# marksgraham/ddpm-ood

Measured on AMD Instinct MI355X. Metric: reconstructions/sec (whole node), FashionMNIST 32x32, higher is better.
Workload: dtype f32 (split-f16 MFMA products, fp32 accumulate)

## Files before the change

ddpm_ood_amd/csrc/conv_direct.hip:

```cpp
#include <stdlib.h>

#include "common.h"

namespace ddpm {

template <int COB>
__global__ __launch_bounds__(256) void conv_direct_kernel(const ddpm_conv_desc a) {
  const int HWo = a.Ho * a.Wo, HWi = a.Hi * a.Wi;
  const int Cin = a.C1 + a.C2;
  const int T = a.ksize * a.ksize;
  const int pad = a.ksize == 3 ? 1 : 0;
  const int s = a.mode == DDPM_CONV_STRIDE2 ? 2 : 1;
  const bool up = a.mode == DDPM_CONV_UPSAMPLE2;
  const int Hv = up ? a.Ho : a.Hi, Wv = up ? a.Wo : a.Wi;

  const int p = blockIdx.x * 256 + threadIdx.x;
  const int n = blockIdx.z;
  const int co0 = blockIdx.y * COB;
  if (p >= HWo) return;
  const int ho = p / a.Wo, wo = p - ho * a.Wo;

  float acc[COB];
#pragma unroll
  for (int j = 0; j < COB; ++j) acc[j] = 0.f;

  for (int ci = 0; ci < Cin; ++ci) {
    const float *plane = (ci < a.C1) ? a.in1 + ((size_t)n * a.C1 + ci) * HWi
                                     : a.in2 + ((size_t)n * a.C2 + (ci - a.C1)) * HWi;
    float sc = 1.f, sh = 0.f;
    if (a.gscale) {
      sc = a.gscale[(size_t)n * Cin + ci];
      sh = a.gshift[(size_t)n * Cin + ci];
    }
    for (int kh = 0; kh < a.ksize; ++kh) {
      for (int kw = 0; kw < a.ksize; ++kw) {
        const int hv = ho * s + kh - pad, wv = wo * s + kw - pad;
        float v = 0.f;
        if (hv >= 0 && hv < Hv && wv >= 0 && wv < Wv) {
          v = up ? plane[(hv >> 1) * a.Wi + (wv >> 1)] : plane[hv * a.Wi + wv];
          if (a.gscale) v = v * sc + sh;
          if (a.act == DDPM_ACT_SILU) v = silu_fast(v);
          if (a.act == DDPM_ACT_RELU) v = fmaxf(v, 0.f);
        }
        const int t = kh * a.ksize + kw;
#pragma unroll
        for (int j = 0; j < COB; ++j) {
          const int co = (co0 + j < a.Cout) ? co0 + j : a.Cout - 1;
          acc[j] = fmaf(v, a.w_raw[((size_t)co * Cin + ci) * T + t], acc[j]);
        }
      }
    }
  }
#pragma unroll
  for (int j = 0; j < COB; ++j) {
    const int co = co0 + j;
    if (co < a.Cout) {
      const size_t idx = ((size_t)n * a.Cout + co) * HWo + p;
      float v = acc[j];
      if (a.bias) v += a.bias[co];
      if (a.chan_add) v += a.chan_add[(size_t)n * a.chan_add_stride + co];
      if (a.residual) v += a.residual[idx];
      if (a.out_act == DDPM_ACT_RELU) v = fmaxf(v, 0.f);
      a.out[idx] = v;
    }
  }
}

constexpr int kSC_CH = 8;

template <int NPOS>
__global__ __launch_bounds__(256) void conv_smallco_kernel(const ddpm_conv_desc a, int TH, int RS, int PS) {
  extern __shared__ __attribute__((aligned(16))) float tile[];
  const int HW = a.Ho * a.Wo;
  const int Cin = a.C1 + a.C2;
  const int tid = threadIdx.x;
  const int n = blockIdx.y;
  const int h0 = blockIdx.x * TH;
  const bool live = tid < TH * a.Wo;
  const int th = live ? tid / a.Wo : 0, tw = live ? tid - th * a.Wo : 0;

  int soff[NPOS];
#pragma unroll
  for (int j = 0; j < NPOS; ++j) {
    const int r = tid + 256 * j;
    soff[j] = -1;
    if (r < PS) {
      const int ir = r / RS, ic = r - ir * RS;
      const int hv = h0 + ir - 1, wv = ic - 1;
      if (hv >= 0 && hv < a.Hi && wv >= 0 && wv < a.Wi) soff[j] = hv * a.Wi + wv;
    }
  }
  float acc[4] = {0.f, 0.f, 0.f, 0.f};
  const int pix = th * RS + tw;

  float pre[NPOS][kSC_CH], psc[kSC_CH], psh[kSC_CH];
  auto fetch = [&](int c0) {
#pragma unroll
    for (int c = 0; c < kSC_CH; ++c) {
      const int ci = c0 + c;
      const bool okc = ci < Cin;
      const float *plane = !okc ? a.in1
                           : (ci < a.C1) ? a.in1 + ((size_t)n * a.C1 + ci) * HW
                                         : a.in2 + ((size_t)n * a.C2 + (ci - a.C1)) * HW;
#pragma unroll
      for (int j = 0; j < NPOS; ++j) pre[j][c] = (okc && soff[j] >= 0) ? plane[soff[j]] : 0.f;
      psc[c] = (okc && a.gscale) ? a.gscale[(size_t)n * Cin + ci] : 1.f;
      psh[c] = (okc && a.gscale) ? a.gshift[(size_t)n * Cin + ci] : 0.f;
    }
  };
  fetch(0);
  for (int c0 = 0; c0 < Cin; c0 += kSC_CH) {
    __syncthreads();
#pragma unroll
    for (int j = 0; j < NPOS; ++j) {
      const int r = tid + 256 * j;
      if (r < PS) {
#pragma unroll
        for (int c = 0; c < kSC_CH; ++c) {
          float v = 0.f;
          if (soff[j] >= 0 && c0 + c < Cin) {
            v = pre[j][c];
            if (a.gscale) v = v * psc[c] + psh[c];
            if (a.act == DDPM_ACT_SILU) v = silu_fast(v);
            if (a.act == DDPM_ACT_RELU) v = fmaxf(v, 0.f);
          }
          tile[c * PS + r] = v;
        }
      }
    }
    __syncthreads();
    if (c0 + kSC_CH < Cin) fetch(c0 + kSC_CH);
#pragma unroll
    for (int c = 0; c < kSC_CH; ++c) {
      const int ci = c0 + c;
      if (ci < Cin) {
        float x[9];
#pragma unroll
        for (int kh = 0; kh < 3; ++kh)
#pragma unroll
          for (int kw = 0; kw < 3; ++kw) x[kh * 3 + kw] = tile[c * PS + pix + kh * RS + kw];
        for (int co = 0; co < a.Cout; ++co) {
          const float *w = a.w_raw + ((size_t)co * Cin + ci) * 9;
#pragma unroll
          for (int t = 0; t < 9; ++t) acc[co] = fmaf(x[t], w[t], acc[co]);
        }
      }
    }
  }
  const int p = (h0 + th) * a.Wo + tw;
  for (int co = 0; co < a.Cout && live; ++co) {
    const size_t idx = ((size_t)n * a.Cout + co) * HW + p;
    float v = acc[co];
    if (a.bias) v += a.bias[co];
    if (a.chan_add) v += a.chan_add[(size_t)n * a.chan_add_stride + co];
    if (a.residual) v += a.residual[idx];
    if (a.out_act == DDPM_ACT_RELU) v = fmaxf(v, 0.f);
    a.out[idx] = v;
  }
}

constexpr int kSW_NJ = 7;
constexpr int kSW_PPL = 4;

template <int NWV>
__global__ __launch_bounds__(64 * NWV) void conv_smallco_wave_kernel(const ddpm_conv_desc a, int TH, int RS, int PS) {
  extern __shared__ __attribute__((aligned(16))) float lds[];
  const int HW = a.Ho * a.Wo;
  const int Cin = a.C1 + a.C2;
  const int tid = threadIdx.x, lane = tid & 63, wave = __builtin_amdgcn_readfirstlane(tid >> 6);
  const int n = blockIdx.y;
  const int h0 = blockIdx.x * TH;
  float *plane_lds = lds + wave * 2 * PS;

  int soff[kSW_NJ];
#pragma unroll
  for (int j = 0; j < kSW_NJ; ++j) {
    const int r = lane + 64 * j;
    soff[j] = -1;
    if (r < PS) {
      const int ir = r / RS, ic = r - ir * RS;
      const int hv = h0 + ir - 1, wv = ic - 1;
      if (hv >= 0 && hv < a.Hi && wv >= 0 && wv < a.Wi) soff[j] = hv * a.Wi + wv;
    }
  }
  int pix[kSW_PPL];
#pragma unroll
  for (int k = 0; k < kSW_PPL; ++k) {
    const int q = lane + 64 * k;
    const int th = q / a.Wo, tw = q - th * a.Wo;
    pix[k] = (q < TH * a.Wo) ? th * RS + tw : 0;
  }
  float acc[kSW_PPL][4];
#pragma unroll
  for (int k = 0; k < kSW_PPL; ++k)
#pragma unroll
    for (int c = 0; c < 4; ++c) acc[k][c] = 0.f;

  float pre[2][kSW_NJ], psc[2] = {1.f, 1.f}, psh[2] = {0.f, 0.f};
  auto fetch = [&](int slot, int ci) {
    const float *plane = (ci < a.C1) ? a.in1 + ((size_t)n * a.C1 + ci) * HW
                                     : a.in2 + ((size_t)n * a.C2 + (ci - a.C1)) * HW;
#pragma unroll
    for (int j = 0; j < kSW_NJ; ++j) pre[slot][j] = soff[j] >= 0 ? plane[soff[j]] : 0.f;
    if (a.gscale) {
      psc[slot] = a.gscale[(size_t)n * Cin + ci];
      psh[slot] = a.gshift[(size_t)n * Cin + ci];
    }
  };
  auto consume = [&](int slot, int ci, int buf) {
    float *pl = plane_lds + buf * PS;
#pragma unroll
    for (int j = 0; j < kSW_NJ; ++j) {
      const int r = lane + 64 * j;
      if (r < PS) {
        float v = 0.f;
        if (soff[j] >= 0) {
          v = pre[slot][j];
          if (a.gscale) v = v * psc[slot] + psh[slot];
          if (a.act == DDPM_ACT_SILU) v = silu_fast(v);
          if (a.act == DDPM_ACT_RELU) v = fmaxf(v, 0.f);
        }
        pl[r] = v;
      }
    }
    if (ci + 2 * NWV < Cin) fetch(slot, ci + 2 * NWV);
    float wreg[4][9];
#pragma unroll
    for (int co = 0; co < 4; ++co) {
      const float *w = a.w_raw + ((size_t)min(co, a.Cout - 1) * Cin + ci) * 9;
#pragma unroll
      for (int t = 0; t < 9; ++t) wreg[co][t] = w[t];
    }
#pragma unroll
    for (int k = 0; k < kSW_PPL; ++k) {
      float x[9];
#pragma unroll
      for (int kh = 0; kh < 3; ++kh)
#pragma unroll
        for (int kw = 0; kw < 3; ++kw) x[kh * 3 + kw] = pl[pix[k] + kh * RS + kw];
#pragma unroll
      for (int co = 0; co < 4; ++co)
        if (co < a.Cout) {
#pragma unroll
          for (int t = 0; t < 9; ++t) acc[k][co] = fmaf(x[t], wreg[co][t], acc[k][co]);
        }
    }
  };
  if (wave < Cin) fetch(0, wave);
  if (wave + NWV < Cin) fetch(1, wave + NWV);
  for (int ci = wave; ci < Cin; ci += 2 * NWV) {
    consume(0, ci, 0);
    if (ci + NWV < Cin) consume(1, ci + NWV, 1);
  }
  float *red = lds + NWV * 2 * PS;
#pragma unroll
  for (int k = 0; k < kSW_PPL; ++k)
#pragma unroll
    for (int c = 0; c < 4; ++c) red[(wave * 256 + lane + 64 * k) * 4 + c] = acc[k][c];
  __syncthreads();
  if (tid < TH * a.Wo) {
    const int th = tid / a.Wo, tw = tid - th * a.Wo;
    const int p = (h0 + th) * a.Wo + tw;
    for (int co = 0; co < a.Cout; ++co) {
      float v = red[(0 * 256 + tid) * 4 + co];
#pragma unroll
      for (int wv = 1; wv < NWV; ++wv) v += red[(wv * 256 + tid) * 4 + co];
      const size_t idx = ((size_t)n * a.Cout + co) * HW + p;
      if (a.bias) v += a.bias[co];
      if (a.chan_add) v += a.chan_add[(size_t)n * a.chan_add_stride + co];
      if (a.residual) v += a.residual[idx];
      if (a.out_act == DDPM_ACT_RELU) v = fmaxf(v, 0.f);
      a.out[idx] = v;
    }
  }
}

template <int CIN>
__global__ __launch_bounds__(256) void conv_smallci_kernel(const ddpm_conv_desc a) {
  const int HW = a.Ho * a.Wo;
  const int p = blockIdx.x * 256 + threadIdx.x;
  const int n = blockIdx.y;
  if (p >= HW) return;
  const int ho = p / a.Wo, wo = p - ho * a.Wo;
  float x[CIN * 9];
#pragma unroll
  for (int ci = 0; ci < CIN; ++ci) {
    const float *plane = a.in1 + ((size_t)n * CIN + ci) * HW;
#pragma unroll
    for (int kh = 0; kh < 3; ++kh)
#pragma unroll
      for (int kw = 0; kw < 3; ++kw) {
        const int hv = ho + kh - 1, wv = wo + kw - 1;
        x[ci * 9 + kh * 3 + kw] = (hv >= 0 && hv < a.Hi && wv >= 0 && wv < a.Wi) ? plane[hv * a.Wi + wv] : 0.f;
      }
  }
  float *dst = a.out + (size_t)n * a.Cout * HW + p;
  const int cpz = (a.Cout + gridDim.z - 1) / gridDim.z, co_end = min(a.Cout, ((int)blockIdx.z + 1) * cpz);
  extern __shared__ float2 wred[];
  const bool emit = a.stats_out != nullptr;
  const int lane = threadIdx.x & 63, wave = threadIdx.x >> 6;
#pragma unroll 4
  for (int co = blockIdx.z * cpz; co < co_end; ++co) {
    const float *w = a.w_raw + (size_t)co * CIN * 9;
    float acc = 0.f;
#pragma unroll
    for (int k = 0; k < CIN * 9; ++k) acc = fmaf(x[k], w[k], acc);
    if (a.bias) acc += a.bias[co];
    dst[(size_t)co * HW] = acc;
    if (emit) {
      const float mean = wave_sum_dpp_last_lane(acc);
      const float mu = __builtin_bit_cast(float, __builtin_amdgcn_readlane(__builtin_bit_cast(int, mean), 63)) * (1.f / 64.f);
      const float dv = acc - mu;
      const float q = wave_sum_dpp_last_lane(dv * dv);
      if (lane == 63) wred[(co - blockIdx.z * cpz) * 4 + wave] = make_float2(mu, q);
    }
  }
  if (emit) {
    __syncthreads();
    const int parts = HW / 256;
    for (int c = threadIdx.x; c < co_end - (int)blockIdx.z * cpz; c += 256) {
      const float2 w0 = wred[c * 4], w1 = wred[c * 4 + 1], w2 = wred[c * 4 + 2], w3 = wred[c * 4 + 3];
      const float m01 = 0.5f * (w0.x + w1.x), d01 = w1.x - w0.x, q01 = (w0.y + w1.y) + d01 * d01 * 32.f;
      const float m23 = 0.5f * (w2.x + w3.x), d23 = w3.x - w2.x, q23 = (w2.y + w3.y) + d23 * d23 * 32.f;
      const float mm = 0.5f * (m01 + m23), dd = m23 - m01, qq = (q01 + q23) + dd * dd * 64.f;
      const int co = blockIdx.z * cpz + c;
      *reinterpret_cast<float2 *>(a.stats_out + (((size_t)n * a.Cout + co) * parts + blockIdx.x) * 2) = make_float2(mm, qq);
    }
  }
}

static bool smallci_supported(const ddpm_conv_desc &d) {
  const bool on = sw().convin_fast;
  return on && d.C2 == 0 && d.C1 >= 1 && d.C1 <= 4 && d.ksize == 3 && d.mode == DDPM_CONV_NORMAL && !d.gscale &&
         d.act == DDPM_ACT_NONE && !d.chan_add && !d.residual && d.out_act == DDPM_ACT_NONE && d.Cout >= 16 &&
         d.Di <= 1 && d.Do <= 1 && d.dims != 3;
}

static int smallci_stats_parts(const ddpm_conv_desc &d) {
  const int HW = d.Ho * d.Wo;
  if (!smallci_supported(d) || HW % 256 || HW / 256 > 8) return 0;
  return HW / 256;
}

static bool smallco_supported(const ddpm_conv_desc &d, int &TH, int &RS, int &PS) {
  if (d.Cout > 4 || d.ksize != 3 || d.mode != DDPM_CONV_NORMAL || d.Wo > 256 || d.Di > 1 || d.Do > 1) return false;
  TH = 0;
  for (int th = 256 / d.Wo; th >= 1; --th)
    if (d.Ho % th == 0) { TH = th; break; }
  if (TH == 0 || 2 * TH * d.Wo < 256) return false;
  RS = d.Wo + 2;
  PS = (TH + 2) * RS;
  return PS <= 512;
}

int launch_conv_direct(const ddpm_conv_desc &d, hipStream_t s) {
  DDPM_CHECK_ARG(d.w_raw != nullptr, "conv_direct: w_raw is NULL");
  DDPM_CHECK_ARG(d.ksize == 1 || d.ksize == 3, "conv_direct: ksize must be 1 or 3");
  DDPM_CHECK_ARG(d.B <= 65535, "conv_direct: batch > 65535");
  const int HWo = d.Ho * d.Wo;
  const double cin = d.C1 + d.C2, taps = d.ksize * d.ksize;
  const int Cin_i = d.C1 + d.C2;
  int TH, RS, PS;
  if (smallco_supported(d, TH, RS, PS)) {
    ProfScope prof(s, "conv3x3_small_cout", 2.0 * d.B * HWo * d.Cout * cin * 9,
                   4.0 * ((double)d.B * cin * HWo + (double)d.B * HWo * d.Cout + d.Cout * cin * 9));
    dim3 grid(d.Ho / TH, d.B);
    const bool wave_ok = sw().convout_wave;
    if (wave_ok && PS <= 64 * kSW_NJ && Cin_i >= 16) {
      const long w16_max = sw().convout_w16_maxwg;
      const long w16_wgs = w16_max >= 0 ? w16_max : 2L * device_cus();
      if ((long)grid.x * grid.y <= w16_wgs && Cin_i >= 64) {
        const size_t lds_w = ((size_t)16 * 2 * PS + 16 * 256 * 4) * sizeof(float);
        static bool attr_done = false;
        if (!attr_done) {
          (void)hipFuncSetAttribute(reinterpret_cast<const void *>(&conv_smallco_wave_kernel<16>), hipFuncAttributeMaxDynamicSharedMemorySize, 160 * 1024);
          attr_done = true;
        }
        hipLaunchKernelGGL(conv_smallco_wave_kernel<16>, grid, dim3(1024), lds_w, s, d, TH, RS, PS);
        DDPM_CHECK_LAUNCH();
        return 0;
      }
      const size_t lds_w = ((size_t)4 * 2 * PS + 4 * 256 * 4) * sizeof(float);
      hipLaunchKernelGGL(conv_smallco_wave_kernel<4>, grid, dim3(256), lds_w, s, d, TH, RS, PS);
      DDPM_CHECK_LAUNCH();
      return 0;
    }
    const size_t lds = (size_t)kSC_CH * PS * sizeof(float);
    if (PS <= 256)
      hipLaunchKernelGGL(conv_smallco_kernel<1>, grid, dim3(256), lds, s, d, TH, RS, PS);
    else
      hipLaunchKernelGGL(conv_smallco_kernel<2>, grid, dim3(256), lds, s, d, TH, RS, PS);
    DDPM_CHECK_LAUNCH();
    return 0;
  }
  if (smallci_supported(d)) {
    ProfScope prof(s, "conv3x3_small_cin", 2.0 * d.B * HWo * d.Cout * cin * 9,
                   4.0 * ((double)d.B * cin * HWo + (double)d.B * HWo * d.Cout + d.Cout * cin * 9));
    const long blocks = (long)((HWo + 255) / 256) * d.B;
    int zs = 1;
    const long zblk = sw().convin_blocks_per_cu;
    while (zs < 8 && blocks * zs * 2 <= device_cus() * zblk && d.Cout / (zs * 2) >= 16) zs *= 2;
    dim3 grid((HWo + 255) / 256, d.B, zs);
    ddpm_conv_desc dk = d;
    if (smallci_stats_parts(d) == 0) dk.stats_out = nullptr;
    const size_t lds = dk.stats_out ? (size_t)((d.Cout + zs - 1) / zs) * 4 * sizeof(float2) : 0;
    switch (d.C1) {
      case 1: hipLaunchKernelGGL(conv_smallci_kernel<1>, grid, dim3(256), lds, s, dk); break;
      case 2: hipLaunchKernelGGL(conv_smallci_kernel<2>, grid, dim3(256), lds, s, dk); break;
      case 3: hipLaunchKernelGGL(conv_smallci_kernel<3>, grid, dim3(256), lds, s, dk); break;
      default: hipLaunchKernelGGL(conv_smallci_kernel<4>, grid, dim3(256), lds, s, dk); break;
    }
    DDPM_CHECK_LAUNCH();
    return 0;
  }
  ProfScope prof(s, "conv_direct", 2.0 * d.B * HWo * d.Cout * cin * taps,
                 4.0 * ((double)d.B * cin * d.Hi * d.Wi + (double)d.B * HWo * d.Cout * (d.residual ? 2 : 1) +
                        d.Cout * cin * taps));
  if (d.Cout <= 4) {
    dim3 grid((HWo + 255) / 256, d.Cout, d.B);
    hipLaunchKernelGGL(conv_direct_kernel<1>, grid, dim3(256), 0, s, d);
  } else {
    dim3 grid((HWo + 255) / 256, (d.Cout + 7) / 8, d.B);
    hipLaunchKernelGGL(conv_direct_kernel<8>, grid, dim3(256), 0, s, d);
  }
  DDPM_CHECK_LAUNCH();
  return 0;
}

bool conv_direct_supported(const ddpm_conv_desc &) { return true; }

int conv_direct_stats_parts(const ddpm_conv_desc &d) {
  int TH, RS, PS;
  return d.mode == DDPM_CONV_NORMAL && !smallco_supported(d, TH, RS, PS) ? smallci_stats_parts(d) : 0;
}

}
```

Baseline: 1058.

## Add quad-pixel small-Cin conv kernel with LDS weights and per-wave channel split

Adds a new kernel for the 3x3 small-input-channel conv (the network's input layer). Each lane computes four adjacent output pixels from a register-held 3x6 input window. The block's output channels are split across its four waves, and weights plus bias are staged in LDS. The aim is to reuse input loads across pixels and channels and to store with float4. Per-channel mean/variance stats are reduced inside one wave over 256 pixels, which removes the cross-wave LDS merge. The cost is more registers per thread and reliance on Wo being a multiple of 4.

```diff
diff --git a/ddpm_ood_amd/csrc/conv_direct.hip b/ddpm_ood_amd/csrc/conv_direct.hip
--- a/ddpm_ood_amd/csrc/conv_direct.hip
+++ b/ddpm_ood_amd/csrc/conv_direct.hip
@@ -325,6 +325,92 @@
       const float mm = 0.5f * (m01 + m23), dd = m23 - m01, qq = (q01 + q23) + dd * dd * 64.f;
       const int co = blockIdx.z * cpz + c;
       *reinterpret_cast<float2 *>(a.stats_out + (((size_t)n * a.Cout + co) * parts + blockIdx.x) * 2) = make_float2(mm, qq);
+    }
+  }
+}
+
+template <int CIN>
+__global__ __launch_bounds__(256) void conv_smallci_quad_kernel(const ddpm_conv_desc a) {
+  constexpr int K = CIN * 9;
+  constexpr int U = CIN == 1 ? 4 : CIN == 2 ? 2 : 1;
+  const int HW = a.Ho * a.Wo;
+  const int lane = threadIdx.x & 63, wave = __builtin_amdgcn_readfirstlane(threadIdx.x >> 6);
+  const int p = blockIdx.x * 256 + 4 * lane;
+  const int n = blockIdx.y;
+  const int cpz = (a.Cout + gridDim.z - 1) / gridDim.z, z0 = blockIdx.z * cpz, z_end = min(a.Cout, z0 + cpz);
+  extern __shared__ __attribute__((aligned(16))) float wlds[];
+  for (int i = threadIdx.x; i < (z_end - z0) * (K + 1); i += 256) {
+    const int c = i / (K + 1), k = i - c * (K + 1);
+    wlds[i] = k < K ? a.w_raw[(size_t)(z0 + c) * K + k] : (a.bias ? a.bias[z0 + c] : 0.f);
+  }
+  __syncthreads();
+  if (p >= HW) return;
+  const int ho = p / a.Wo, wo = p - ho * a.Wo;
+  float x[CIN][3][6];
+#pragma unroll
+  for (int ci = 0; ci < CIN; ++ci) {
+    const float *plane = a.in1 + ((size_t)n * CIN + ci) * HW;
+#pragma unroll
+    for (int kh = 0; kh < 3; ++kh)
+#pragma unroll
+      for (int c = 0; c < 6; ++c) {
+        const int hv = ho + kh - 1, wv = wo + c - 1;
+        const bool ok = hv >= 0 && hv < a.Hi && wv >= 0 && wv < a.Wi;
+        const float v = plane[ok ? hv * a.Wi + wv : p];
+        x[ci][kh][c] = ok ? v : 0.f;
+      }
+  }
+  const int cpw = (z_end - z0 + 3) / 4, co0 = z0 + wave * cpw, co_end = min(z_end, co0 + cpw);
+  if (co0 >= co_end) return;
+  float *dst = a.out + (size_t)n * a.Cout * HW + p;
+  const bool emit = a.stats_out != nullptr;
+  const int parts = HW / 256;
+  for (int co = co0; co < co_end; co += U) {
+    float wc[U][K], bc[U];
+#pragma unroll
+    for (int u = 0; u < U; ++u) {
+      const float *w = wlds + (min(co + u, co_end - 1) - z0) * (K + 1);
+#pragma unroll
+      for (int k = 0; k < K; ++k) wc[u][k] = w[k];
+      bc[u] = w[K];
+    }
+    float acc[U][4];
+#pragma unroll
+    for (int u = 0; u < U; ++u)
+#pragma unroll
+      for (int j = 0; j < 4; ++j) {
+        float v = 0.f;
+#pragma unroll
+        for (int ci = 0; ci < CIN; ++ci)
+#pragma unroll
+          for (int kh = 0; kh < 3; ++kh)
+#pragma unroll
+            for (int kw = 0; kw < 3; ++kw) v = fmaf(x[ci][kh][j + kw], wc[u][ci * 9 + kh * 3 + kw], v);
+        if (a.bias) v += bc[u];
+        acc[u][j] = v;
+      }
+#pragma unroll
+    for (int u = 0; u < U; ++u)
+      if (co + u < co_end)
+        *reinterpret_cast<float4 *>(dst + (size_t)(co + u) * HW) = make_float4(acc[u][0], acc[u][1], acc[u][2], acc[u][3]);
+    if (emit) {
+      float mu[U], q[U];
+#pragma unroll
+      for (int u = 0; u < U; ++u) {
+        const float t = wave_sum_dpp_last_lane((acc[u][0] + acc[u][1]) + (acc[u][2] + acc[u][3]));
+        mu[u] = __builtin_bit_cast(float, __builtin_amdgcn_readlane(__builtin_bit_cast(int, t), 63)) * (1.f / 256.f);
+      }
+#pragma unroll
+      for (int u = 0; u < U; ++u) {
+        const float d0 = acc[u][0] - mu[u], d1 = acc[u][1] - mu[u], d2 = acc[u][2] - mu[u], d3 = acc[u][3] - mu[u];
+        q[u] = wave_sum_dpp_last_lane((d0 * d0 + d1 * d1) + (d2 * d2 + d3 * d3));
+      }
+      if (lane == 63) {
+#pragma unroll
+        for (int u = 0; u < U; ++u)
+          if (co + u < co_end)
+            *reinterpret_cast<float2 *>(a.stats_out + (((size_t)n * a.Cout + co + u) * parts + blockIdx.x) * 2) = make_float2(mu[u], q[u]);
+      }
     }
   }
 }
@@ -403,6 +489,17 @@
     dim3 grid((HWo + 255) / 256, d.B, zs);
     ddpm_conv_desc dk = d;
     if (smallci_stats_parts(d) == 0) dk.stats_out = nullptr;
+    const size_t wl = (size_t)((d.Cout + zs - 1) / zs) * (d.C1 * 9 + 1) * sizeof(float);
+    if (d.Wo % 4 == 0 && wl <= 48 * 1024) {
+      switch (d.C1) {
+        case 1: hipLaunchKernelGGL(conv_smallci_quad_kernel<1>, grid, dim3(256), wl, s, dk); break;
+        case 2: hipLaunchKernelGGL(conv_smallci_quad_kernel<2>, grid, dim3(256), wl, s, dk); break;
+        case 3: hipLaunchKernelGGL(conv_smallci_quad_kernel<3>, grid, dim3(256), wl, s, dk); break;
+        default: hipLaunchKernelGGL(conv_smallci_quad_kernel<4>, grid, dim3(256), wl, s, dk); break;
+      }
+      DDPM_CHECK_LAUNCH();
+      return 0;
+    }
     const size_t lds = dk.stats_out ? (size_t)((d.Cout + zs - 1) / zs) * 4 * sizeof(float2) : 0;
     switch (d.C1) {
       case 1: hipLaunchKernelGGL(conv_smallci_kernel<1>, grid, dim3(256), lds, s, dk); break;
```

Result: no change. 1064 (median of 6 runs) (+0.6%).
